# chairclr/PathTracing

Measured on AMD Instinct MI355X. Metric: Mrays/s, higher is better.
Workload: dtype f32

## Files before the change

### pathtracing_amd/csrc/kernels.hip

```cpp
#include "ptrt_internal.h"
#include "pt_device.h"
#include <algorithm>
#include <cstdlib>
#include <type_traits>

using namespace ptd;

namespace ptrt {

PT_DEV uint32_t lane_prefix(uint64_t m) { return __builtin_amdgcn_mbcnt_hi((uint32_t)(m >> 32), __builtin_amdgcn_mbcnt_lo((uint32_t)m, 0u)); }
PT_DEV uint32_t lane_id() { return lane_prefix(~0ull); }

typedef const float4 __attribute__((address_space(4))) *uniform_f4;
PT_DEV uniform_f4 as_uniform(const float4 *p) { return (uniform_f4)(uintptr_t)p; }
PT_DEV float4 uniform_load(uniform_f4 p, uint32_t i) { return make_float4(p[i].x, p[i].y, p[i].z, p[i].w); }
PT_DEV uint32_t spheres_test(const float4 *spheres, uint32_t n_spheres, uint32_t first_id, V3 o, V3 d, Hit &h)
{
    const uniform_f4 sp = as_uniform(spheres);
    for (uint32_t j = 0; j < n_spheres; j += 4u) {
        const float4 s0 = uniform_load(sp, j), s1 = uniform_load(sp, j + 1u), s2 = uniform_load(sp, j + 2u), s3 = uniform_load(sp, j + 3u);
        sphere_test(s0, first_id + j, o, d, h);
        if (j + 1u < n_spheres) sphere_test(s1, first_id + j + 1u, o, d, h);
        if (j + 2u < n_spheres) sphere_test(s2, first_id + j + 2u, o, d, h);
        if (j + 3u < n_spheres) sphere_test(s3, first_id + j + 3u, o, d, h);
// ... 484 lines not shown
            float s;
            const float4 tx = ea.texels[env_texel(ea, d, s)];
            V3 e = xyz(tx);
            if constexpr (NEE)
                if (ea.lit && nr->aux > 0.0f) {
                    const float w = mis_weight(env_pdf(ea, tx, s) / nr->aux);
                    e = v3(tx.x * w, tx.y * w, tx.z * w);
                }
            add(e);
        } else
        add(v3(sc.sky[0], sc.sky[1], sc.sky[2]));
        term = true;
    } else {
        const V3 P = madd(t, d, o);
        V3 ng;
        uint32_t mat;
        if (ref < sc.n_tris) {
            const float4 ts = sc.tris[(size_t)ref * 4 + 3];
            ng = xyz(ts);
            mat = __float_as_uint(ts.w);
        } else {
            const uint32_t j = ref - sc.n_tris;
            const float4 s = sc.spheres[j];
            const uint2 mi = sc.sph_mat[j];
            const float ir = __uint_as_float(mi.y);
            ng = v3((P.x - s.x) * ir, (P.y - s.y) * ir, (P.z - s.z) * ir);
            mat = mi.x;
        }
        const bool front = dot(ng, d) < 0.0f;
        const V3 n = front ? ng : neg(ng);
        float4 m0 = sc.mats[(size_t)mat * 3], m1 = sc.mats[(size_t)mat * 3 + 1];
        const float4 m2 = sc.mats[(size_t)mat * 3 + 2];
        asm volatile("" : "+v"(m0.x), "+v"(m1.x));
        const V3 alb = v3(m0.y, m0.z, m0.w), emi = xyz(m1);
        const uint32_t kind = __float_as_uint(m0.x);
        if (MODE == SHADE_QUEUE && kind != (uint32_t)PT_LAMBERT) { defer = 1u + kind; return false; }
        if (emi.x != 0.0f || emi.y != 0.0f || emi.z != 0.0f) {
            if constexpr (NEE) {
                V3 e = emi;
                if (nr->aux > 0.0f && ref < sc.n_tris && (!ENV || kernargs<true, ENV>().nee.n_lights)) {
                    float pa = kernargs<true, ENV>().nee.pa[ref];
                    if constexpr (ENV) pa = pa * kernargs<NEE, true>().env.psel;
                    if (pa > 0.0f) {
                        const float pl = (pa * (t * t)) / __builtin_fabsf(dot(ng, d)), w = mis_weight(pl / nr->aux);
                        e = v3(emi.x * w, emi.y * w, emi.z * w);
                    }
                }
                add(e);
            } else add(emi);
        }
        if (depth >= fp.max_depth) term = true;
        else {
            const uint32_t bb = depth - 1u;
            const uint32_t bk = MODE == SHADE_QUEUE ? (uint32_t)B_LAMBERT : MODE == SHADE_BUCKETS ? b : 1u + kind;
            if (SHARED && bk == B_LAMBERT) {
                T = v3(T.x * alb.x, T.y * alb.y, T.z * alb.z);
                if (roulette_ends(fp, key, depth, bb, T)) term = true;
                if (!term) { o = madd(fp.ray_eps, n, P); d = n; lambert = true; }
            } else {
                BsdfSample bs;
                if (bk == B_LAMBERT) bs = sample_lambert(alb, n, u01(key, 4u + 4u * bb), u01(key, 5u + 4u * bb));
                else if (bk == B_METAL) bs = sample_metal(alb, m1.w, d, n, u01(key, 4u + 4u * bb), u01(key, 5u + 4u * bb));
                else bs = sample_dielectric(alb, m2.x, d, n, front, u01(key, 6u + 4u * bb));
                const V3 wi = bs.wi, W = bs.W;
                const float side = bs.side;
                V3 ta = T;
                if (!bs.ok) term = true;
                else {
                    T = v3(T.x * W.x, T.y * W.y, T.z * W.z);
                    ta = T;
                    if (roulette_ends(fp, key, depth, bb, T)) term = true;
                    if (!term) { o = madd(side * fp.ray_eps, n, P); d = wi; }
                }
                if constexpr (NEE) {
                    const NeeArgs &na = kernargs<true, ENV>().nee;
                    auto lights = [&]() -> bool {
                        if constexpr (ENV) return na.n_lights || kernargs<NEE, true>().env.lit;
                        else return na.n_lights;
                    };
                    if (!term) nr->aux = (bk == B_LAMBERT && lights()) ? dot(n, wi) * kInvPi : 0.0f;
                    if (bk == B_LAMBERT && lights()) {
                        float uc = 0.0f;
                        bool to_env = false;
                        if constexpr (ENV) {
                            uc = u01(key, 1024u + 3u * bb);
                            to_env = kernargs<NEE, true>().env.lit != 0u;
                            if (to_env && na.n_lights) { to_env = uc < 0.5f; uc = to_env ? uc * 2.0f : fma_(uc, 2.0f, -1.0f); }
                        }
                        if (ENV && to_env) {
                            const EnvArgs &ea = kernargs<NEE, true>().env;
                            const uint32_t j = pick_light(ea.mcdf, ea.n, uc), i = pick_light(ea.ccdf + (size_t)j * ea.n, ea.n, u01(key, 1025u + 3u * bb));
                            const float u = fma_((float)i + u01(key, 1026u + 3u * bb), ea.step, -1.0f), v = fma_((float)j + u01(key, 2048u + bb), ea.step, -1.0f);
                            const V3 wl = env_decode(u, v);
                            float s;
                            const float4 tx = ea.texels[env_texel(ea, wl, s)];
                            const float cs = dot(n, wl), pl = env_pdf(ea, tx, s);
                            if (cs > 0.0f && pl > 0.0f) {
                                const float f = mis_weight_times_q((cs * kInvPi) / pl);
                                at(na.rad, slot) = make_float4((ta.x * f) * tx.x, (ta.y * f) * tx.y, (ta.z * f) * tx.z, 0.0f);
                                if (!term) at(na.ext, slot) = make_float4(d.x, d.y, d.z, nr->aux);
                                nr->flags = NEE_PENDING | (term ? NEE_END : 0u);
                                nr->aux = __builtin_inff();
                                o = madd(fp.ray_eps, n, P); d = wl;
                                term = false;
                            }
                        } else {
                        const float4 *lr = na.lights + (size_t)pick_light(na.cdf, na.n_lights, ENV ? uc : u01(key, 1024u + 3u * bb)) * 4;
                        const float4 l0 = lr[0], l1 = lr[1], l2 = lr[2];
                        const float su = __builtin_sqrtf(u01(key, 1025u + 3u * bb)), b1 = 1.0f - su, b2 = u01(key, 1026u + 3u * bb) * su;
                        const V3 x = v3(fma_(b2, l2.x, fma_(b1, l1.x, l0.x)), fma_(b2, l2.y, fma_(b1, l1.y, l0.y)), fma_(b2, l2.z, fma_(b1, l1.z, l0.z)));
                        const V3 so = madd(fp.ray_eps, n, P);
                        const V3 dl = x - so;
                        const float dist2 = dot(dl, dl), dist = __builtin_sqrtf(dist2), inv = 1.0f / dist;
                        const V3 sd = v3(dl.x * inv, dl.y * inv, dl.z * inv);
                        const float4 l3 = lr[3];
                        const float cs = dot(n, sd), cl = __builtin_fabsf(dot(xyz(l3), sd));
                        if (cs > 0.0f && cl > 0.0f) {
                            float pa = l0.w;
                            if constexpr (ENV) pa = pa * kernargs<NEE, true>().env.psel;
                            const float pl = (pa * dist2) / cl, f = mis_weight_times_q((cs * kInvPi) / pl);
                            at(na.rad, slot) = make_float4((ta.x * f) * l1.w, (ta.y * f) * l2.w, (ta.z * f) * l3.w, 0.0f);
                            if (!term) at(na.ext, slot) = make_float4(d.x, d.y, d.z, nr->aux);
                            nr->flags = NEE_PENDING | (term ? NEE_END : 0u);
                            nr->aux = dist * 0.9999f;
                            o = so; d = sd;
                            term = false;
                        }
                        }
                    }
                }
            }
        }
    }

    uint32_t x = 0, y = 0;
    if (term) {
        touched = true;
        A.w += 1.0f;
        sample += fp.streams;
        if (sample < fp.spp) {
            slot_pixel(slot, fp, x, y);
            if constexpr (LENS) camera_sample<true, true>(sc, fp, x, y, r, depth, &lens_args<NEE, ENV>());
            else
            camera_sample<!SHARED>(sc, fp, x, y, r, depth);
            regen = SHARED; alive = true;
        }
        if constexpr (NEE) nr->aux = 0.0f;
    } else alive = true;
    if (lambert || regen) {
        const uint32_t dim = regen ? 0u : 4u * depth;
        float u1 = u01(key, dim), u2 = u01(key, dim + 1u);
        V3 v;
        if (regen) {
            if (!sc.cam.jitter) u1 = u2 = 0.5f;
            v = camera_vec_of(sc.cam, x, y, u1, u2);
        } else v = lambert_vec(d, u1, u2);
        d = normalize(v);
    }
    if (touched) at(ps.acc, slot) = A;
    r.depth = depth;
    return alive;
}

template <bool LENS = false>
PT_DEV bool resolve_shadow(const DeviceScene &sc, const PathState &ps, const FrameParams &fp, const NeeArgs &na, uint32_t slot, PathRegs &r,
                           NeeRegs &nr, bool visible, const LensArgs *lens = nullptr)
{
    const bool end = (nr.flags & NEE_END) != 0u;
    bool alive = true;
    if (visible || end) {
        float4 A = at(ps.acc, slot);
        if (visible) { const float4 L = at(na.rad, slot); A.x = A.x + L.x; A.y = A.y + L.y; A.z = A.z + L.z; }
        if (end) { A.w += 1.0f; alive = next_sample<LENS>(sc, fp, slot, r, r.depth, lens); nr.aux = 0.0f; }
        at(ps.acc, slot) = A;
    }
    if (!end) { const float4 e = at(na.ext, slot); r.d = xyz(e); nr.aux = e.w; }
    nr.flags = 0u;
    return alive;
}

PT_DEV unsigned long long *traced_counter(const PathState &ps, uint32_t c, uint32_t shard)
{
    return reinterpret_cast<unsigned long long *>(ps.counters + cnt_traced_index(c, shard));
}
PT_DEV void fold_traced(const PathState &ps, uint32_t shard, uint32_t it, uint32_t n, uint32_t n_alive)
{
    *traced_counter(ps, (it + 2u) % 3u, shard) = 0ull;
    const unsigned long long traced = *traced_counter(ps, it % 3u, shard);
    *reinterpret_cast<unsigned long long *>(ps.counters + cnt_rays_index(shard)) += traced;
    if (ps.host_ring && it) ps.host_ring[((it - 1u) % ps.ring_slots) * kShards + shard] = make_uint4(n, n_alive, (uint32_t)traced, (uint32_t)(traced >> 32));
}

PT_DEV bool want_compact(const PathState &ps, uint32_t len, uint32_t n_alive, uint32_t prev_alive, bool sticky, bool forced)
{
    const uint32_t deaths = prev_alive > n_alive ? prev_alive - n_alive : 0u;
    const uint32_t predicted = n_alive > deaths ? n_alive - deaths : 0u;
    return forced || (sticky && len < ps.shard_cap) || (float)predicted < ps.compact_below * (float)len;
}

PT_DEV void queue_next(const PathState &ps, uint32_t shard, uint32_t cnext, uint32_t *q_next, uint32_t gid, uint32_t total, bool alive,
                       uint32_t slot, bool compact)
{
    if (compact) wave_push(&ps.counters[cnt_ext_index(cnext, shard)], q_next, alive, slot);
    else {
        if (gid < total) at(q_next, gid) = alive ? slot : kInvalidSlot;
        if (gid == 0) ps.counters[cnt_ext_index(cnext, shard)] = total;
    }
    const uint64_t m = __ballot(alive);
    if (m && lane_id() == 0u) atomicAdd(&ps.counters[cnt_alive_index(cnext, shard)], (uint32_t)__popcll(m));
}

#ifndef PT_EXT_WAVES
#define PT_EXT_WAVES(L, FUSE) (((L) == PT_BVH_WIDTH_4Q || (L) == PT_BVH_WIDTH_2) && (FUSE) != SHADE_INLINE ? 8 : 7)
#endif
#ifndef PT_EXT_WAVES_NEE
#define PT_EXT_WAVES_NEE(L, FUSE) ((FUSE) == SHADE_QUEUE && (L) != PT_BVH_WIDTH_8Q && (L) != PT_BVH_WIDTH_8O ? 7 : 6)
#endif
#define PT_EXT_WAVES_OF(L, FUSE, NEE) ((NEE) ? PT_EXT_WAVES_NEE(L, FUSE) : PT_EXT_WAVES(L, FUSE))
#ifndef PT_EXT_WAVES_ENV
#define PT_EXT_WAVES_ENV(L, NEE) ((NEE) ? 5 : (L) == PT_BVH_WIDTH_8O ? 6 : 7)
#endif
#define PT_EXT_WAVES_FOR(L, FUSE, NEE, ENV) ((ENV) ? PT_EXT_WAVES_ENV(L, NEE) : PT_EXT_WAVES_OF(L, FUSE, NEE))
#ifndef PT_EXT_WAVES_LENS
#define PT_EXT_WAVES_LENS(L, NEE, ENV) (!(NEE) && ((L) == PT_BVH_WIDTH_8Q || (L) == PT_BVH_WIDTH_8O) ? 6 : PT_EXT_WAVES_FOR(L, SHADE_INLINE, NEE, ENV))
#endif
#define PT_EXT_WAVES_K(L, FUSE, NEE, ENV) ((FUSE) == 3  ? PT_EXT_WAVES_LENS(L, NEE, ENV) : PT_EXT_WAVES_FOR(L, FUSE, NEE, ENV))
struct StackCtx { int32_t *lds; uint32_t stride, tid, col; };
PT_DEV void push_slow(const StackCtx &k, uint32_t &sp, int32_t v)
{
    if (sp < kStackLds) k.lds[sp * k.stride + k.tid] = v;
    else {
        const PathState &ps = cold().ps;
        const uint32_t e = sp - kStackLds;
        if (e < ps.stack_ovf_entries) ps.stack_ovf[(size_t)e * ((size_t)kShards * ps.shard_cap) + k.col] = v;
        else { atomicOr(&ps.counters[kCntError], 1u); return; }
    }
    ++sp;
}
PT_DEV int32_t pop_slow(const StackCtx &k, uint32_t &sp)
{
    if (sp == 0) return PT_BVH_EMPTY;
    --sp;
    if (sp < kStackLds) return k.lds[sp * k.stride + k.tid];
    const PathState &ps = cold().ps;
    return ps.stack_ovf[(size_t)(sp - kStackLds) * ((size_t)kShards * ps.shard_cap) + k.col];
}
PT_DEV int32_t pop_lds(const StackCtx &k, uint32_t &sp)
{
    if (sp == 0) return PT_BVH_EMPTY;
    --sp;
    return k.lds[sp * k.stride + k.tid];
}
PT_DEV int32_t pop_after_leaf(const StackCtx &k, uint32_t &sp)
{
    const bool deep = __any((int)(sp > kStackLds)) != 0;
    return deep ? pop_slow(k, sp) : pop_lds(k, sp);
}

template <int L, VisitOrder ORD>
PT_DEV void node_visit_rows(const float4 *__restrict__ base, float4 r0, float4 r1, float4 r2, float4 r3, const StackCtx &k, const RaySetup &rs,
                            float t_best, int32_t &cur, uint32_t &sp);
template <int ROWS>
PT_DEV const float4 *record(const float4 *base, uint32_t i)
{
    return reinterpret_cast<const float4 *>(reinterpret_cast<const char *>(base) + (size_t)(i * (uint32_t)(ROWS * 16)));
}
template <int L, VisitOrder ORD>
PT_DEV void node_step(const float4 *__restrict__ nodes, const StackCtx &k, const RaySetup &rs, float t_best, int32_t &cur, uint32_t &sp)
{
    const float4 *base = record<node_rows<L>()>(nodes, (uint32_t)cur);
    node_visit_rows<L, ORD>(base, base[0], base[1], base[2], base[3], k, rs, t_best, cur, sp);
}
template <int L, VisitOrder ORD>
PT_DEV void node_visit_rows(const float4 *__restrict__ base, float4 r0, float4 r1, float4 r2, float4 r3, const StackCtx &k, const RaySetup &rs,
                            float t_best, int32_t &cur, uint32_t &sp)
{
    constexpr int N = fanout<L>();
    const bool deep = __any((int)(sp + (uint32_t)(N - 1) > kStackLds)) != 0;
    if constexpr (L == PT_BVH_WIDTH_8O) {
        uint32_t hits;
        int32_t ref[N];
        visit_node_oct8(base, r0, r1, r2, r3, rs, t_best, hits, ref);
        int32_t prev = PT_BVH_EMPTY;
        if (!deep) {
#pragma unroll
            for (int p = N - 1; p >= 0; --p) {
                const bool h = (hits >> p) & 1u;
                k.lds[sp * k.stride + k.tid] = prev;
                sp += (h && prev != PT_BVH_EMPTY) ? 1u : 0u;
                prev = h ? ref[p] : prev;
            }
            cur = prev != PT_BVH_EMPTY ? prev : pop_lds(k, sp);
        } else {
#pragma unroll
            for (int p = N - 1; p >= 0; --p)
                if ((hits >> p) & 1u) { if (prev != PT_BVH_EMPTY) push_slow(k, sp, prev); prev = ref[p]; }
            cur = prev != PT_BVH_EMPTY ? prev : pop_slow(k, sp);
        }
        return;
    }
    uint32_t key[N];
    int32_t ref[N];
    visit_node<L, ORD>(base, r0, r1, r2, r3, rs, t_best, key, ref);
    if (!deep) {
#pragma unroll
        for (int i = N - 1; i >= 1; --i) {
            k.lds[sp * k.stride + k.tid] = ref[i];
            sp += key[i] != 0xFFFFFFFFu ? 1u : 0u;
        }
        cur = key[0] != 0xFFFFFFFFu ? ref[0] : pop_lds(k, sp);
    } else {
#pragma unroll
        for (int i = N - 1; i >= 1; --i)
            if (key[i] != 0xFFFFFFFFu) push_slow(k, sp, ref[i]);
        cur = (key[0] != 0xFFFFFFFFu) ? ref[0] : pop_slow(k, sp);
    }
}

PT_DEV uint32_t leaf_step(const float4 *__restrict__ tris, const StackCtx &k, V3 o, V3 d, Hit &h, int32_t &cur, uint32_t &sp)
{
    const uint32_t enc = (uint32_t)~cur;
    uint32_t first = enc >> 3, more = enc & 7u, n = 0;
    for (;;) {
        const float4 *base = record<4>(tris, first);
        const float4 r0 = base[0], r1 = base[1], r2 = base[2];
        tri_test(r0, r1, r2, first, o, d, h);
        ++n;
        if (more == 0u) break;
        ++first; --more;
    }
    cur = pop_after_leaf(k, sp);
    return n;
}
PT_DEV void leaf_step_any(const float4 *__restrict__ tris, const StackCtx &k, V3 o, V3 d, Hit &h, int32_t &cur, uint32_t &sp)
{
    const uint32_t enc = (uint32_t)~cur;
    uint32_t first = enc >> 3, more = enc & 7u;
    for (;;) {
        const float4 *base = tris + (size_t)first * 4;
        tri_test(base[0], base[1], base[2], first, o, d, h);
        if (h.id != PT_MISS) { cur = PT_BVH_EMPTY; return; }
        if (more == 0u) break;
        ++first; --more;
    }
    cur = pop_after_leaf(k, sp);
}

constexpr uint32_t kFinishVertices = 256;

struct ExtHead {
    uint32_t shard, bx, parity, cnext, n, n_alive;
    bool do_compact, idle;
};
template <int FUSE>
PT_DEV ExtHead extend_head(const ExtArgs &a, const PathState &ps, uint32_t per_block, uint32_t tid, bool predicted, bool carry_len)
{
    ExtHead e;
    const uint32_t it = a.it, ccur = it % 3u, czero = (it + 2u) % 3u;
    e.parity = it & 1u; e.cnext = (it + 1u) % 3u;
    uint32_t nbx;
    block_pos(a.ps, e.shard, e.bx, nbx);
    e.n = ps.counters[cnt_ext_index(ccur, e.shard)]; e.n_alive = ps.counters[cnt_alive_index(ccur, e.shard)];
    e.do_compact = FUSE != SHADE_NONE &&
                   (predicted ? want_compact(ps, e.n, e.n_alive, ps.counters[cnt_prev_alive_index(ccur, e.shard)], ps.repack_sticky != 0u, a.compact != 0u)
                              : want_compact(ps, e.n, e.n_alive, 0u, false, a.compact != 0u));
    if (e.bx * per_block + tid == 0u) {
        ps.counters[cnt_prev_alive_index(e.cnext, e.shard)] = e.n_alive;
        ps.counters[cnt_ext_index(czero, e.shard)] = 0u;
        ps.counters[cnt_alive_index(czero, e.shard)] = 0u;
        fold_traced(ps, e.shard, it, e.n, e.n_alive);
        if (FUSE == SHADE_NONE) *traced_counter(ps, e.cnext, e.shard) = e.n_alive;
        else if (carry_len && !e.do_compact) ps.counters[cnt_ext_index(e.cnext, e.shard)] = e.n;
        if (e.do_compact && e.n_alive) atomicAdd(&ps.counters[kCntCompactions], 1u);
    }
    e.idle = e.bx * per_block >= e.n || e.n_alive == 0u;
    return e;
}

PT_DEV void stash_park(uint32_t *stash, uint32_t stride, uint32_t tid, const PathRegs &r)
{
    stash[0 * stride + tid] = __float_as_uint(r.T.x); stash[1 * stride + tid] = __float_as_uint(r.T.y);
    stash[2 * stride + tid] = __float_as_uint(r.T.z); stash[3 * stride + tid] = r.key;
    stash[4 * stride + tid] = (r.sample << 8) | r.depth;
    asm volatile("" ::: "memory");
}
PT_DEV void stash_restore(const uint32_t *stash, uint32_t stride, uint32_t tid, PathRegs &r)
{
    r.T = v3(__uint_as_float(stash[0 * stride + tid]), __uint_as_float(stash[1 * stride + tid]), __uint_as_float(stash[2 * stride + tid]));
    r.key = stash[3 * stride + tid];
    const uint32_t sdv = stash[4 * stride + tid];
    r.sample = sdv >> 8; r.depth = sdv & 255u;
}

struct VisitCounts {
    unsigned long long nodes = 0, tris = 0, sph = 0;
    unsigned long long wave_iters = 0, wave_iters_late = 0, idle_leaf = 0, idle_done = 0;
};
PT_DEV void flush_visit_counters(const PathState &ps, const VisitCounts &v)
{
    auto add = [&](uint32_t i, unsigned long long x) { atomicAdd(reinterpret_cast<unsigned long long *>(ps.counters + i), x); };
    if (v.wave_iters) add(kCntWaveNodeIters, v.wave_iters);
    if (v.wave_iters_late) add(kCntWaveNodeIters + 2, v.wave_iters_late);
    if (v.idle_leaf) add(kCntIdleLeaf, v.idle_leaf);
    if (v.idle_done) add(kCntIdleDone, v.idle_done);
    add(kCntNodes, v.nodes);
    add(kCntTris, v.tris);
    add(kCntSph, v.sph);
}

template <int L, bool COUNT, bool DIAG, bool ANY>
PT_DEV Hit trace_ray(const HotScene &g, const StackCtx &stk, V3 o, V3 d, Hit h, VisitCounts &vc, int32_t *s_state)
{
    constexpr VisitOrder ORD = visit_order<L, COUNT>();
    { const uint32_t ns = spheres_test(g, o, d, h); if (COUNT) vc.sph += ns; }

    const RaySetup rs = ray_setup(o, d);
    int32_t cur = PT_BVH_EMPTY;
    uint32_t sp = 0, steps = 0;
    if (g.n_nodes && !(ANY && h.id != PT_MISS)) {
        ++steps;
        if (COUNT) vc.nodes++;
        if (DIAG && lane_id() == (uint32_t)(__ffsll((long long)__ballot(1)) - 1)) vc.wave_iters++;
        const uniform_f4 root = as_uniform(g.nodes);
        node_visit_rows<L, ORD>(g.nodes, uniform_load(root, 0), uniform_load(root, 1), uniform_load(root, 2), uniform_load(root, 3), stk, rs, h.t, cur, sp);
        if (DIAG) s_state[stk.tid & 63u] = cur;
    }

    bool late_cycle = false;
    for (;;) {
        while ((uint32_t)cur < (uint32_t)PT_BVH_EMPTY) {
            if (++steps > (1u << 22)) { atomicOr(&cold().ps.counters[kCntError], 2u); cur = PT_BVH_EMPTY; break; }
            if (COUNT) vc.nodes++;
            if (DIAG && lane_id() == (uint32_t)(__ffsll((long long)__ballot(1)) - 1)) {
                vc.wave_iters++; if (late_cycle) vc.wave_iters_late++;
                uint32_t n_leaf = 0, n_done = 0;
                for (uint32_t l = 0; l < 64u; ++l) { const int32_t c2 = s_state[l]; n_leaf += c2 < 0 ? 1u : 0u; n_done += c2 == PT_BVH_EMPTY ? 1u : 0u; }
                vc.idle_leaf += n_leaf; vc.idle_done += n_done;
            }
            node_step<L, ORD>(g.nodes, stk, rs, h.t, cur, sp);
            if (DIAG) s_state[stk.tid & 63u] = cur;
        }
        if (cur == PT_BVH_EMPTY) break;
        if (DIAG) late_cycle = true;
        if (ANY) leaf_step_any(g.tris, stk, o, d, h, cur, sp);
        else { const uint32_t nt = leaf_step(g.tris, stk, o, d, h, cur, sp); if (COUNT) vc.tris += nt; }
        if (DIAG) s_state[stk.tid & 63u] = cur;
    }
    return h;
}

constexpr int FUSE_LENS = 3;
template <int L, bool COUNT, int FUSE_, bool NEE = false, bool ENV = false>
__global__ void __launch_bounds__(kExtBlock) __attribute__((amdgpu_waves_per_eu(PT_EXT_WAVES_K(L, FUSE_, NEE, ENV), PT_EXT_WAVES_K(L, FUSE_, NEE, ENV))))
k_extend(std::conditional_t<FUSE_ == FUSE_LENS, ExtLensArgsT<NEE, ENV>, ExtArgsT<NEE, ENV>> args)
{
    constexpr bool LENS = FUSE_ == FUSE_LENS;
    constexpr int FUSE = LENS ? (int)SHADE_INLINE : FUSE_;
    const ExtArgs &a = ext_of(args);
    static_assert(!NEE || (FUSE != SHADE_NONE && !COUNT), "NEE: fused shading, no visit counters");
    static_assert(!ENV || (FUSE == SHADE_INLINE && !COUNT), "ENV: all-kinds fused shading, no visit counters");
    static_assert(!LENS || (FUSE == SHADE_INLINE && !COUNT), "LENS: all-kinds fused shading, no visit counters");
    const HotScene g = hot_scene(a.sc);
    const uint32_t it = a.it;
    __shared__ int32_t s_stack[kStackLds * kExtBlock];
    __shared__ uint32_t s_stash[(FUSE != SHADE_NONE ? (NEE ? 7 : 5) : 1) * kExtBlock];
    const uint32_t tid = threadIdx.x;
    ExtHead hd;
    uint32_t gid, qbase, slot = kInvalidSlot, n_bounces;
    {
        const PathState &ps = cold().ps;
        hd = extend_head<FUSE>(a, ps, kExtBlock, tid, true, false);
        gid = hd.bx * kExtBlock + tid;
        if (hd.idle) return;
        qbase = hd.shard * ps.shard_cap;
        if (gid < hd.n) slot = at(ps.q_ext[hd.parity], qbase + gid);
        if (FUSE != SHADE_NONE) slot = queued_slot(it, slot);
        const bool sparse = hd.do_compact && (float)hd.n_alive < ps.sparse_below * (float)hd.n;
        n_bounces = FUSE == SHADE_NONE ? 1u : (hd.n_alive <= ps.finish_below ? kFinishVertices : sparse ? 1u : a.bounces);
    }
    const uint32_t shard = hd.shard, parity = hd.parity, n = hd.n;
    const bool active = slot != kInvalidSlot;
    const StackCtx stk{ s_stack, kExtBlock, tid, qbase + gid };

    VisitCounts vc;
    __shared__ int32_t s_state[COUNT ? 64 : 1];
    PathRegs r = path_none();
    NeeRegs nr{ 0.0f, 0u };
    if (active) {
        if (FUSE == SHADE_NONE) { const PathState &ps = cold().ps; r.o = xyz(at(ps.ray_o, slot)); r.d = xyz(at(ps.ray_d, slot)); }
        else if constexpr (LENS) path_begin<NEE, true>(it, slot, r, &nr, &lens_args<NEE, ENV>());
        else path_begin<NEE>(it, slot, r, &nr);
    }
    bool alive = active;
    uint32_t wave_rays = 0;
    for (uint32_t bounce = 0; bounce < n_bounces; ++bounce) {
        const uint64_t alive_mask = __ballot(alive);
        if (alive_mask == 0) break;
        wave_rays += (uint32_t)__popcll(alive_mask);
        if (COUNT && kExtBlock == 64u) { s_state[tid] = alive ? 0 : 1; __syncthreads(); }
        if (alive) {
            const V3 o = r.o, d = r.d;
            Hit h{ (NEE && (nr.flags & NEE_PENDING)) ? nr.aux : __builtin_inff(), PT_MISS, PT_MISS };
            if (FUSE != SHADE_NONE) stash_park(s_stash, kExtBlock, tid, r);
            if constexpr (NEE) {
                s_stash[5 * kExtBlock + tid] = __float_as_uint(nr.aux); s_stash[6 * kExtBlock + tid] = nr.flags;
                asm volatile("" ::: "memory");
            }
            h = trace_ray<L, COUNT, COUNT, false>(g, stk, o, d, h, vc, s_state);
            if (FUSE == SHADE_NONE) at(cold().ps.hit, slot) = make_float2(h.t, __uint_as_float(h.ref));
            else {
                stash_restore(s_stash, kExtBlock, tid, r);
                uint32_t defer = 0u;
                const ExtArgs &c = cold();
                if constexpr (NEE) {
                    nr.aux = __uint_as_float(s_stash[5 * kExtBlock + tid]); nr.flags = s_stash[6 * kExtBlock + tid];
                    if (nr.flags & NEE_PENDING) {
                        if constexpr (LENS) alive = resolve_shadow<true>(c.sc, c.ps, c.fp, kernargs<true, ENV>().nee, slot, r, nr, h.ref == PT_MISS, &lens_args<true, ENV>());
                        else alive = resolve_shadow(c.sc, c.ps, c.fp, kernargs<true, ENV>().nee, slot, r, nr, h.ref == PT_MISS);
                    } else alive = shade_one<FUSE, true, ENV, LENS>(c.sc, c.ps, c.fp, slot, r, h.t, h.ref, B_LAMBERT, defer, &nr);
                } else alive = shade_one<FUSE, false, ENV, LENS>(c.sc, c.ps, c.fp, slot, r, h.t, h.ref, B_LAMBERT, defer);
            }
        }
    }
    const PathState &ps = cold().ps;
    if (COUNT && active) flush_visit_counters(ps, vc);
    if (FUSE != SHADE_NONE) {
        if (alive) path_store<NEE>(ps, slot, r, &nr);
        queue_next(ps, shard, hd.cnext, &at(ps.q_ext[parity ^ 1u], qbase), gid, n, alive, slot, hd.do_compact);
        if (wave_rays && lane_id() == 0u) atomicAdd(traced_counter(ps, hd.cnext, shard), (unsigned long long)wave_rays);
    }
}

#ifndef PT_REFILL_IDLE
#define PT_REFILL_IDLE 16
#endif
constexpr uint32_t kRefillIdle = PT_REFILL_IDLE;

#ifndef PT_PACKED_WAVES
#define PT_PACKED_WAVES(FUSE) ((FUSE) == SHADE_INLINE ? 6 : 7)
#endif
template <int L, bool COUNT, int FUSE>
__global__ void __launch_bounds__(64) __attribute__((amdgpu_waves_per_eu(PT_PACKED_WAVES(FUSE), PT_PACKED_WAVES(FUSE))))
k_extend_packed(ExtArgs a)
{
    const float4 *__restrict__ nodes = a.sc.nodes, *__restrict__ tris = a.sc.tris, *__restrict__ spheres = a.sc.spheres;
    const uint32_t n_spheres = a.sc.n_spheres, n_tris = a.sc.n_tris, n_nodes = a.sc.n_nodes;
    const uint32_t it = a.it, chunk = a.chunk, bounces = a.bounces;
    __shared__ int32_t s_stack[kStackLds * 64];
    __shared__ uint32_t s_stash[(FUSE != SHADE_NONE ? 5 : 1) * 64];
    const uint32_t lane = threadIdx.x;
    const ExtHead hd = extend_head<FUSE>(a, cold().ps, chunk, lane, false, true);
    if (hd.idle) return;
    const uint32_t shard = hd.shard, n_alive = hd.n_alive;
    const bool do_compact = hd.do_compact;
    uint32_t next = hd.bx * chunk;
    const uint32_t end = min(hd.n, next + chunk);
    const uint32_t qbase = hd.shard * cold().ps.shard_cap;
    const uint32_t *queue = cold().ps.q_ext[hd.parity] + (size_t)qbase;
    uint32_t *q_next = cold().ps.q_ext[hd.parity ^ 1u] + (size_t)qbase;
    const StackCtx stk{ s_stack, 64u, lane, qbase + hd.bx * 64u + lane };
    const uint32_t budget0 = FUSE == SHADE_NONE ? 1u : (n_alive <= cold().ps.finish_below ? kFinishVertices : bounces);

    bool has = false;
    uint32_t slot = 0, pos = 0, budget = 0, sp = 0, steps = 0;
    int32_t cur = PT_BVH_EMPTY;
    PathRegs r = path_none();
    V3 &o = r.o, &d = r.d;
    RaySetup rs = ray_setup(o, d);
    Hit h{ __builtin_inff(), PT_MISS, PT_MISS };
    VisitCounts vc;
    uint32_t wave_rays = 0, wave_alive = 0;

    auto start_ray = [&]() {
        if (FUSE != SHADE_NONE) stash_park(s_stash, 64u, lane, r);
        h = Hit{ __builtin_inff(), PT_MISS, PT_MISS };
        { const uint32_t ns = spheres_test(spheres, n_spheres, n_tris, o, d, h); if (COUNT) vc.sph += ns; }
        rs = ray_setup(o, d);
        cur = n_nodes ? 0 : PT_BVH_EMPTY;
        sp = 0; steps = 0;
    };

    for (;;) {
        const bool fin = has && cur == PT_BVH_EMPTY;
        bool retired = false, retire_alive = false;
        if (fin) {
            if (FUSE == SHADE_NONE) {
                at(cold().ps.hit, slot) = make_float2(h.t, __uint_as_float(h.ref));
                has = false;
            } else {
                stash_restore(s_stash, 64u, lane, r);
                uint32_t defer = 0u;
                const bool alive = shade_one<FUSE>(cold().sc, cold().ps, cold().fp, slot, r, h.t, h.ref, B_LAMBERT, defer);
                --budget;
                if (alive && budget != 0u) start_ray();
                else {
                    if (alive) path_store(cold().ps, slot, r);
                    retired = true; retire_alive = alive; has = false;
                }
            }
        }
        if (FUSE != SHADE_NONE) {
            wave_rays += (uint32_t)__popcll(__ballot(fin && has));
            wave_alive += (uint32_t)__popcll(__ballot(retire_alive));
            if (do_compact) wave_push(&cold().ps.counters[cnt_ext_index(hd.cnext, shard)], q_next, retire_alive, slot);
            else if (retired) q_next[pos] = retire_alive ? slot : kInvalidSlot;
        }
        const uint64_t idle = __ballot(!has);
        const uint32_t avail = end - next;
        if (idle && avail) {
            const uint32_t prefix = lane_prefix(idle);
            const bool pull = !has && prefix < avail;
            if (pull) { pos = next + prefix; slot = queue[pos]; if (FUSE != SHADE_NONE) slot = queued_slot(it, slot); }
            if (pull && slot == kInvalidSlot) {
                if (FUSE != SHADE_NONE && !do_compact) q_next[pos] = kInvalidSlot;
            } else if (pull) {
                if (FUSE == SHADE_NONE) { o = xyz(at(cold().ps.ray_o, slot)); d = xyz(at(cold().ps.ray_d, slot)); }
                else path_begin(it, slot, r);
                budget = budget0;
                start_ray();
                has = true;
            }
            if (FUSE != SHADE_NONE) wave_rays += (uint32_t)__popcll(__ballot(pull && has));
            next += min((uint32_t)__popcll(idle), avail);
        }
        if (!__ballot(has)) {
            if (next < end) continue;
            break;
        }
        const uint32_t want = (next < end) ? kRefillIdle : 64u;
        for (;;) {
            if (cur != PT_BVH_EMPTY) {
                const bool inner = cur >= 0;
                const uint32_t enc = (uint32_t)~cur, first = enc >> 3, more = enc & 7u;
                const float4 *base = inner ? nodes + (size_t)cur * node_rows<L>() : tris + (size_t)first * 4;
                const float4 r0 = base[0], r1 = base[1], r2 = base[2], r3 = base[3];
                if (++steps > (1u << 22)) { atomicOr(&cold().ps.counters[kCntError], 2u); cur = PT_BVH_EMPTY; }
                else if (inner) {
                    node_visit_rows<L, ORDER_SPEC>(base, r0, r1, r2, r3, stk, rs, h.t, cur, sp);
                    if (COUNT) vc.nodes++;
                } else {
                    tri_test(r0, r1, r2, first, o, d, h);
                    if (COUNT) vc.tris++;
                    cur = more ? (int32_t)~(((first + 1u) << 3) | (more - 1u)) : pop_after_leaf(stk, sp);
                }
            }
            const uint32_t busy = (uint32_t)__popcll(__ballot(has && cur != PT_BVH_EMPTY));
            if (FUSE == SHADE_NONE) { if (busy == 0u || 64u - busy >= want) break; }
            else {
                const uint32_t waiting = (uint32_t)__popcll(__ballot(has && cur == PT_BVH_EMPTY));
                const uint32_t empty = (next < end) ? (uint32_t)__popcll(__ballot(!has)) : 0u;
                if (busy == 0u || waiting + empty >= kRefillIdle) break;
            }
        }
    }
    if (COUNT) flush_visit_counters(cold().ps, vc);
    if (FUSE != SHADE_NONE && lane == 0u) {
        if (wave_rays) atomicAdd(traced_counter(cold().ps, hd.cnext, shard), (unsigned long long)wave_rays);
        if (wave_alive) atomicAdd(&cold().ps.counters[cnt_alive_index(hd.cnext, shard)], wave_alive);
    }
}

#ifndef PT_POOL_WAVES
#define PT_POOL_WAVES(FUSE) ((FUSE) == SHADE_INLINE ? 6 : 7)
#endif
#ifndef PT_POOL_REFILL
#define PT_POOL_REFILL 16
#endif
#ifndef PT_POOL_LEAFWAIT
#define PT_POOL_LEAFWAIT 16
#endif
constexpr uint32_t kPoolRefill = PT_POOL_REFILL, kPoolLeafWait = PT_POOL_LEAFWAIT;

template <int L, bool COUNT, int FUSE>
__global__ void __launch_bounds__(64) __attribute__((amdgpu_waves_per_eu(PT_POOL_WAVES(FUSE), PT_POOL_WAVES(FUSE)))) k_extend_pool(ExtArgs a)
{
    static_assert(FUSE != SHADE_NONE, "the pool kernel always shades");
    constexpr uint32_t E = kPool, P = E / 64u;
    static_assert(E % 64u == 0 && E >= 64u && E <= 256u, "kPool: 64, 128, 192 or 256 (live list holds byte indices)");
    const float4 *__restrict__ nodes = a.sc.nodes, *__restrict__ tris = a.sc.tris, *__restrict__ spheres = a.sc.spheres;
    const uint32_t n_spheres = a.sc.n_spheres, n_tris = a.sc.n_tris, n_nodes = a.sc.n_nodes;
    __shared__ int32_t s_stack[kStackLds * 64];
    __shared__ float s_ht[E];
    __shared__ uint32_t s_href[E];
    __shared__ uint32_t s_slot[E];
    __shared__ uint8_t s_live[E];
    const uint32_t lane = threadIdx.x;
    ExtHead hd;
    uint32_t n_bounces;
    size_t qbase;
    {
        const PathState &ps = cold().ps;
        hd = extend_head<FUSE>(a, ps, E, lane, true, true);
        if (hd.idle) return;
        qbase = (size_t)hd.shard * ps.shard_cap;
        n_bounces = hd.n_alive <= ps.finish_below ? kFinishVertices : a.bounces;
    }
    const uint32_t shard = hd.shard, bx = hd.bx, parity = hd.parity, n = hd.n;
    const bool do_compact = hd.do_compact;
    const StackCtx stk{ s_stack, 64u, lane, (uint32_t)qbase + bx * 64u + lane };
    VisitCounts vc;

    auto spheres_of = [&](V3 o, V3 d, uint32_t e) {
        Hit h{ __builtin_inff(), PT_MISS, PT_MISS };
        spheres_test(spheres, n_spheres, n_tris, o, d, h);
        s_ht[e] = h.t; s_href[e] = h.ref;
    };
    auto live_append = [&](bool pred, uint32_t e, uint32_t &count) {
        const uint64_t m = __ballot(pred);
        if (pred) s_live[count + lane_prefix(m)] = (uint8_t)e;
        count += (uint32_t)__popcll(m);
    };

    uint32_t n_live = 0;
    {
        const PathState &ps = cold().ps;
#pragma unroll
        for (uint32_t hh = 0; hh < P; ++hh) {
            const uint32_t e = hh * 64u + lane, g = bx * E + e;
            const uint32_t slot = g < n ? ps.q_ext[parity][qbase + g] : kInvalidSlot;
            s_slot[e] = slot;
            const bool valid = slot != kInvalidSlot;
            if (valid) spheres_of(xyz(at(ps.ray_o, slot)), xyz(at(ps.ray_d, slot)), e);
            live_append(valid, e, n_live);
        }
    }
    __syncthreads();

    uint32_t wave_rays = 0;
    for (uint32_t bounce = 0; bounce < n_bounces && n_live; ++bounce) {
        wave_rays += n_live;
// ... 567 lines not shown
```

Measured before the change: 18280.

## Add wave-uniform ballot-driven traversal loop and branchless LDS pop for 4-wide nearest BVH

For non-counting builds, the traversal loop becomes wave-uniform. It is controlled by 64-lane ballots, so all lanes step interior nodes together until none remain, then run leaf processing together. This is meant to cut divergent-branch overhead and keep the SIMD's control flow coherent. For the 4-wide quantized nearest-order BVH, the stack pop on a missed first child becomes a branchless LDS read with a hinted fast path. The trade-off is that lanes finishing interior traversal early may idle while others continue, and the step-limit check changes shape.

```diff
diff --git a/pathtracing_amd/csrc/kernels.hip b/pathtracing_amd/csrc/kernels.hip
--- a/pathtracing_amd/csrc/kernels.hip
+++ b/pathtracing_amd/csrc/kernels.hip
@@ -810,13 +810,22 @@
     uint32_t key[N];
     int32_t ref[N];
     visit_node<L, ORD>(base, r0, r1, r2, r3, rs, t_best, key, ref);
-    if (!deep) {
+    constexpr bool FLAT = ORD == ORDER_NEAREST && L == PT_BVH_WIDTH_4Q;
+    if (FLAT ? __builtin_expect(!deep, 1) : !deep) {
 #pragma unroll
         for (int i = N - 1; i >= 1; --i) {
             k.lds[sp * k.stride + k.tid] = ref[i];
             sp += key[i] != 0xFFFFFFFFu ? 1u : 0u;
         }
-        cur = key[0] != 0xFFFFFFFFu ? ref[0] : pop_lds(k, sp);
+        if constexpr (FLAT) {
+            cur = ref[0];
+            if (key[0] == 0xFFFFFFFFu) {
+                const bool has = sp != 0u;
+                sp -= has ? 1u : 0u;
+                const int32_t top = k.lds[sp * k.stride + k.tid];
+                cur = has ? top : PT_BVH_EMPTY;
+            }
+        } else cur = key[0] != 0xFFFFFFFFu ? ref[0] : pop_lds(k, sp);
     } else {
 #pragma unroll
         for (int i = N - 1; i >= 1; --i)
@@ -934,6 +943,23 @@
         if (DIAG) s_state[stk.tid & 63u] = cur;
     }
 
+    if constexpr (!COUNT) {
+        constexpr uint32_t kMaxSteps = 1u << 22;
+        for (;;) {
+            bool go = (uint32_t)cur < (uint32_t)PT_BVH_EMPTY && steps < kMaxSteps;
+            if (__builtin_amdgcn_ballot_w64(go) != 0) do {
+                if (go) { ++steps; node_step<L, ORD>(g.nodes, stk, rs, h.t, cur, sp); }
+                go = (uint32_t)cur < (uint32_t)PT_BVH_EMPTY && steps < kMaxSteps;
+            } while (__builtin_amdgcn_ballot_w64(go) != 0);
+            if ((uint32_t)cur < (uint32_t)PT_BVH_EMPTY) { atomicOr(&cold().ps.counters[kCntError], 2u); cur = PT_BVH_EMPTY; }
+            if (!__any((int)(cur != PT_BVH_EMPTY))) break;
+            if (cur != PT_BVH_EMPTY) {
+                if (ANY) leaf_step_any(g.tris, stk, o, d, h, cur, sp);
+                else leaf_step(g.tris, stk, o, d, h, cur, sp);
+            }
+        }
+        return h;
+    }
     bool late_cycle = false;
     for (;;) {
         while ((uint32_t)cur < (uint32_t)PT_BVH_EMPTY) {
```

Result: faster. 18560, median of 6 (+1.6%).
